# QData/LaMP

Measured on AMD Instinct MI355X. Metric: forward samples/sec, reuters d512 2+2L 4h, higher is better.
Workload: dtype f32

## Files before the change

lamp_amd/csrc/attention_small.hip:

```cpp
#include "lamp_kernels.h"

namespace lamp {

#ifndef LAMP_LDS_PAD16
#define LAMP_LDS_PAD16 8
#endif
constexpr int ATTN16_PAD = LAMP_LDS_PAD16;

namespace {
__device__ __forceinline__ void swap16(float& a, float& b) {
    asm volatile("s_nop 3\n\tv_permlane16_swap_b32 %0, %1\n\ts_nop 3" : "+v"(a), "+v"(b));
}
__device__ __forceinline__ void swap32(float& a, float& b) {
    asm volatile("s_nop 3\n\tv_permlane32_swap_b32 %0, %1\n\ts_nop 3" : "+v"(a), "+v"(b));
}
__device__ __forceinline__ float group_max(float v) {
    float a = v, b = v;
    swap16(a, b);
    a = fmaxf(a, b);
    b = a;
    swap32(a, b);
    return fmaxf(a, b);
}
__device__ __forceinline__ float group_sum(float v) {
    float a = v, b = v;
    swap16(a, b);
    a = a + b;
    b = a;
    swap32(a, b);
    return a + b;
}
}

template <int DP, int QB, int KSPLIT, int PM, int MK>
__global__ __launch_bounds__(QB* KSPLIT * 64, 3) void attn16_kernel(AttnParams p) {
    constexpr int DKC = DP / 16;
    constexpr int DV8 = DP / 16;
    constexpr int QS = DP + ATTN16_PAD;
    extern __shared__ __attribute__((aligned(16))) float smem[];

    const int tid = threadIdx.x;
    const int lane = tid & 63, wave = tid >> 6;
    const int l15 = lane & 15, g = lane >> 4;
    const int rot = (KSPLIT > 1 && p.kv_len) ? int(blockIdx.x % KSPLIT) : 0;
    const int qb = wave / KSPLIT, ks = __builtin_amdgcn_readfirstlane((wave % KSPLIT + KSPLIT - rot) % KSPLIT);
    const int slot = qb * KSPLIT + ks;
#ifdef LAMP_TUNING
    const unsigned long long t_entry = p.trace ? wall_clock64() : 0ull;
    unsigned long long t_loop = 0, t_merge = 0;
#endif
    const int nqg = (p.lq + 16 * QB - 1) / (16 * QB);
    const int item = xcd_remap(blockIdx.x, gridDim.x);
    const int qgrp = item % nqg;
    const int bh = item / nqg;
    const int h = bh % p.H, b = bh / p.H;
    const int q0 = (qgrp * QB + qb) * 16;
    const int qi = q0 + l15;
    const bool wave_active = q0 < p.lq;
    const int qc = qi < p.lq ? qi : p.lq - 1;

    const int q_r = int(p.lay.q_r), k_r = int(p.lay.k_r), v_r = int(p.lay.v_r);
    const int lk_b = __builtin_amdgcn_readfirstlane(p.kv_len ? p.kv_len[b] : p.lk);
    const int row0 = __builtin_amdgcn_readfirstlane(p.kv_len ? p.kv_off[b] : 0);
    const int64_t k_row0 = p.kv_len ? int64_t(row0) * k_r : int64_t(b) * p.lay.k_b;
    const int64_t v_row0 = p.kv_len ? int64_t(row0) * v_r : int64_t(b) * p.lay.v_b;
    const __amdgpu_buffer_rsrc_t rsQ = make_rsrc(p.Q + int64_t(b) * p.lay.q_b + int64_t(h) * p.lay.q_h,
                                                 (uint64_t(p.lq - 1) * q_r + p.dk) * 4u);
    const __amdgpu_buffer_rsrc_t rsK = make_rsrc(p.K + k_row0 + int64_t(h) * p.lay.k_h,
                                                 lk_b > 0 ? (uint64_t(lk_b - 1) * k_r + p.dk) * 4u : 0);
    const __amdgpu_buffer_rsrc_t rsV = make_rsrc(p.V + v_row0 + int64_t(h) * p.lay.v_h,
                                                 lk_b > 0 ? (uint64_t(lk_b - 1) * v_r + p.dv) * 4u : 0);
    const __amdgpu_buffer_rsrc_t rsM =
        MK == LAMP_MASK_BITS_U32
            ? make_rsrc(static_cast<const unsigned*>(p.mask) + int64_t(b) * p.m_sb,
                        (uint64_t(p.lq - 1) * uint64_t(p.m_sq) + (p.lk + 31) / 32) * 4u)
        : MK == LAMP_MASK_U8
            ? make_rsrc(static_cast<const unsigned char*>(p.mask) + int64_t(b) * p.m_sb,
                        uint64_t(p.lq - 1) * uint64_t(p.m_sq) + p.lk)
        : MK == LAMP_MASK_KEY_TOKENS_I64
            ? make_rsrc(static_cast<const long long*>(p.mask) + int64_t(b) * p.m_sb, uint64_t(p.lk) * 8u)
            : make_rsrc(p.K, 0);

    float* Qs = smem + qb * 16 * QS;
    float* Ks = smem + (QB + wave) * 16 * QS;
    {
        constexpr int C4 = DP / 4;
        constexpr int PER_WAVE = 16 * C4 / KSPLIT;
#pragma unroll
        for (int i = 0; i < (PER_WAVE + 63) / 64; ++i) {
            const int idx = ks * PER_WAVE + i * 64 + lane;
            const int row = idx / C4, c = (idx - row * C4) * 4;
            const int q = q0 + row;
            if (i * 64 + lane < PER_WAVE) {
                const float4 v = bload4(rsQ, (q < p.lq && c < p.dk) ? unsigned(q * q_r + c) * 4u : OOB, 0);
                *reinterpret_cast<float4*>(Qs + row * QS + c) =
                    make_float4(v.x * p.scale_log2e, v.y * p.scale_log2e, v.z * p.scale_log2e, v.w * p.scale_log2e);
            }
        }
    }
    __syncthreads();

    const int nt_b = (lk_b + 15) / 16;
    const int nt = PM == 2 ? (p.lk + 15) / 16 : nt_b;
    const int ks_eff = (KSPLIT > 1 && p.kv_len) ? (nt_b >= 12 ? (KSPLIT < 4 ? KSPLIT : 4) : (nt_b >= 4 ? 2 : 1)) : KSPLIT;
    float4 kg[DKC];
    constexpr int C4K = DP / 4, RPI = 64 / C4K;
    float vf[4][DV8];
    unsigned mbits = 0;

    const unsigned k_voff = (lane % C4K) * 4 < p.dk ? unsigned((lane / C4K) * k_r + (lane % C4K) * 4) * 4u : OOB;
    auto load_k = [&](int kt) {
#pragma unroll
        for (int i = 0; i < DKC; ++i) kg[i] = bload4(rsK, k_voff, unsigned((kt * 16 + i * RPI) * k_r) * 4u);
    };
    auto stage_k = [&]() {
        const int c = (lane % C4K) * 4;
#pragma unroll
        for (int i = 0; i < DKC; ++i) *reinterpret_cast<float4*>(Ks + (i * RPI + lane / C4K) * QS + c) = kg[i];
    };
    constexpr int DVW = DV8 == 8 ? 4 : DV8;
    const unsigned v_voff = DVW * l15 < p.dv ? unsigned(4 * g * v_r + DVW * l15) * 4u : OOB;
    const unsigned v_voff2 = 64 + DVW * l15 < p.dv ? unsigned(4 * g * v_r + DVW * l15) * 4u + 256u : OOB;
    auto load_v = [&](int kt) {
#pragma unroll
        for (int r = 0; r < 4; ++r) {
            const unsigned off = v_voff, so = unsigned((kt * 16 + r) * v_r) * 4u;
            if constexpr (DV8 == 8) {
                const float4 a = bload4(rsV, off, so);
                const float4 c2 = bload4(rsV, v_voff2, so);
                vf[r][0] = a.x; vf[r][1] = a.y; vf[r][2] = a.z; vf[r][3] = a.w;
                vf[r][4] = c2.x; vf[r][5] = c2.y; vf[r][6] = c2.z; vf[r][7] = c2.w;
            } else if constexpr (DV8 == 4) {
                const float4 a = bload4(rsV, off, so);
                vf[r][0] = a.x; vf[r][1] = a.y; vf[r][2] = a.z; vf[r][3] = a.w;
            } else {
                const f32x2 a = bload2(rsV, off + so);
                vf[r][0] = a.x; vf[r][1] = a.y;
            }
        }
    };
    const unsigned m_voff = unsigned(int64_t(qc) * p.m_sq) * 4u;
    auto load_mask = [&](int kt) {
        const int kbase = kt * 16 + 4 * g;
        if constexpr (MK == LAMP_MASK_BITS_U32) {
            mbits = __builtin_amdgcn_raw_buffer_load_b32(rsM, m_voff, unsigned(kt >> 1) * 4u, 0);
        } else if constexpr (MK == LAMP_MASK_U8) {
            const unsigned mo = unsigned(int64_t(qc) * p.m_sq) + unsigned(kbase);
            unsigned m = 0;
#pragma unroll
            for (int r = 0; r < 4; ++r) m |= (bload_u8(rsM, kt < nt ? mo + r : OOB) != 0 ? 1u : 0u) << r;
            mbits = m;
        } else if constexpr (MK == LAMP_MASK_KEY_TOKENS_I64) {
            unsigned m = 0;
#pragma unroll
            for (int r = 0; r < 4; ++r)
                m |= (bload_u64(rsM, unsigned(kbase + r) * 8u) == 0 ? 1u : 0u) << r;
            mbits = m;
        }
    };
    auto scores = [&](int kt, f32x4& s) {
        const int valid = lk_b - kt * 16;
        const unsigned tail = valid >= 16 ? 0u : (0xffffu << (valid > 0 ? valid : 0)) & 0xffffu;
        unsigned word = tail;
        if constexpr (MK == LAMP_MASK_BITS_U32) word |= mbits >> ((kt & 1) * 16);
        const int mine = MK == LAMP_MASK_BITS_U32 || MK == LAMP_MASK_NONE ? int(word >> (4 * g)) : int(mbits | (tail >> (4 * g)));
        f32x4 s0, s1 = {0.f, 0.f, 0.f, 0.f};
#pragma unroll
        for (int r = 0; r < 4; ++r) {
            int t;
            asm("v_bfe_i32 %0, %1, %2, 1" : "=v"(t) : "v"(mine), "n"(r));
            s0[r] = __int_as_float(t & int(0xff800000u));
        }
#ifdef LAMP_SETPRIO
        __builtin_amdgcn_s_setprio(1);
#endif
        const float* qp = Qs + l15 * QS + 4 * g;
        const float* kp = Ks + l15 * QS + 4 * g;
#pragma unroll
        for (int c = 0; c < DKC; c += 2) {
            const float4 qa = *reinterpret_cast<const float4*>(qp + 16 * c);
            const float4 qb2 = *reinterpret_cast<const float4*>(qp + 16 * c + 16);
            const float4 ka = *reinterpret_cast<const float4*>(kp + 16 * c);
            const float4 kb = *reinterpret_cast<const float4*>(kp + 16 * c + 16);
            s0 = __builtin_amdgcn_mfma_f32_16x16x4f32(ka.x, qa.x, s0, 0, 0, 0);
            s1 = __builtin_amdgcn_mfma_f32_16x16x4f32(kb.x, qb2.x, s1, 0, 0, 0);
            s0 = __builtin_amdgcn_mfma_f32_16x16x4f32(ka.y, qa.y, s0, 0, 0, 0);
            s1 = __builtin_amdgcn_mfma_f32_16x16x4f32(kb.y, qb2.y, s1, 0, 0, 0);
            s0 = __builtin_amdgcn_mfma_f32_16x16x4f32(ka.z, qa.z, s0, 0, 0, 0);
            s1 = __builtin_amdgcn_mfma_f32_16x16x4f32(kb.z, qb2.z, s1, 0, 0, 0);
            s0 = __builtin_amdgcn_mfma_f32_16x16x4f32(ka.w, qa.w, s0, 0, 0, 0);
            s1 = __builtin_amdgcn_mfma_f32_16x16x4f32(kb.w, qb2.w, s1, 0, 0, 0);
        }
#ifdef LAMP_SETPRIO
        __builtin_amdgcn_s_setprio(0);
#endif
#pragma unroll
        for (int r = 0; r < 4; ++r) s[r] = s0[r] + s1[r];
    };

    f32x4 o[DV8];
#pragma unroll
    for (int e = 0; e < DV8; ++e) o[e] = f32x4{0.f, 0.f, 0.f, 0.f};
    float m_run = -INFINITY, l_part = 0.f;
    constexpr float RESCALE_THR = 32.0f;

#ifdef LAMP_TUNING
    if (p.trace) t_loop = wall_clock64();
#endif
    if (wave_active && ks < ks_eff && ks < nt) {
        int kt = ks;
        load_k(kt);
        load_mask(kt);
        load_v(kt);
        for (; kt < nt; kt += ks_eff) {
            const int kn = kt + ks_eff;
            f32x4 s;
            stage_k();
            scores(kt, s);
            __builtin_amdgcn_sched_barrier(0);
            load_k(kn);
            load_mask(kn);
            if constexpr (PM == 2) {
                float* Srow = p.P + (int64_t(h) * p.P_batch + p.P_b0 + b) * int64_t(p.lq) * p.lk + int64_t(qi) * p.lk;
#pragma unroll
                for (int r = 0; r < 4; ++r) {
                    const int key = kt * 16 + 4 * g + r;
                    if (qi < p.lq && key < p.lk) Srow[key] = s[r];
                }
            }
            const float tmax = fmaxf(fmaxf(s[0], s[1]), fmaxf(s[2], s[3]));
            if (__any(tmax > m_run + RESCALE_THR)) {
                const float m_new = fmaxf(m_run, group_max(tmax));
                const float alpha = __builtin_amdgcn_exp2f(m_run - ((m_new == -INFINITY) ? 0.f : m_new));
                l_part *= alpha;
                m_run = m_new;
#pragma unroll
                for (int e = 0; e < DV8; ++e)
#pragma unroll
                    for (int r = 0; r < 4; ++r) o[e][r] *= alpha;
            }
            const float m_use = (m_run == -INFINITY) ? 0.f : m_run;
#pragma unroll
            for (int r = 0; r < 4; ++r) s[r] = __builtin_amdgcn_exp2f(s[r] - m_use);
            l_part += (s[0] + s[1]) + (s[2] + s[3]);
#ifdef LAMP_SETPRIO
            __builtin_amdgcn_s_setprio(1);
#endif
#pragma unroll
            for (int r = 0; r < 4; ++r)
#pragma unroll
                for (int e = 0; e < DV8; ++e)
                    o[e] = __builtin_amdgcn_mfma_f32_16x16x4f32(vf[r][e], s[r], o[e], 0, 0, 0);
#ifdef LAMP_SETPRIO
            __builtin_amdgcn_s_setprio(0);
#endif
            __builtin_amdgcn_sched_barrier(0);
            load_v(kn);
        }
    }

#ifdef LAMP_TUNING
    if (p.trace) t_merge = wall_clock64();
#endif
    if constexpr (KSPLIT > 1) {
        constexpr int CW = (DV8 * 4 + 4) * 64;
        __syncthreads();
        float* mine = smem + slot * CW;
#pragma unroll
        for (int e = 0; e < DV8; ++e)
            *reinterpret_cast<float4*>(mine + (e * 64 + lane) * 4) = make_float4(o[e][0], o[e][1], o[e][2], o[e][3]);
        *reinterpret_cast<float4*>(mine + (DV8 * 64 + lane) * 4) = make_float4(m_run, l_part, 0.f, 0.f);
        __syncthreads();
        if (ks == 0 && wave_active) {
            float m_all = m_run;
#pragma unroll
            for (int s2 = 1; s2 < KSPLIT; ++s2)
                if (s2 < ks_eff) m_all = fmaxf(m_all, smem[(slot + s2) * CW + (DV8 * 64 + lane) * 4]);
            const float m_use = (m_all == -INFINITY) ? 0.f : m_all;
            const float w0 = exp2f(m_run - m_use);
            l_part *= w0;
#pragma unroll
            for (int e = 0; e < DV8; ++e)
#pragma unroll
                for (int r = 0; r < 4; ++r) o[e][r] *= w0;
#pragma unroll
            for (int s2 = 1; s2 < KSPLIT; ++s2) {
                if (s2 >= ks_eff) break;
                const float* other = smem + (slot + s2) * CW;
                const float4 ml = *reinterpret_cast<const float4*>(other + (DV8 * 64 + lane) * 4);
                const float ws = exp2f(ml.x - m_use);
                l_part = fmaf(ml.y, ws, l_part);
#pragma unroll
                for (int e = 0; e < DV8; ++e) {
                    const float4 v = *reinterpret_cast<const float4*>(other + (e * 64 + lane) * 4);
                    o[e][0] = fmaf(v.x, ws, o[e][0]);
                    o[e][1] = fmaf(v.y, ws, o[e][1]);
                    o[e][2] = fmaf(v.z, ws, o[e][2]);
                    o[e][3] = fmaf(v.w, ws, o[e][3]);
                }
            }
            m_run = m_all;
        }
    }
    if (!(wave_active && ks == 0)) return;
    const float l_run = group_sum(l_part);
    if constexpr (PM == 2) {
        if (g == 0 && qi < p.lq)
            p.lse[(int64_t(h) * p.B + b) * int64_t(p.lq) + qi] = ((m_run == -INFINITY) ? 0.f : m_run) + log2f(l_run);
    }
    const float inv_l = 1.0f / l_run;

    if (qi < p.lq) {
        float* Orow = p.O + int64_t(b) * p.lay.o_b + int64_t(h) * p.lay.o_h + int64_t(qi) * p.lay.o_r;
        const bool vec = ((p.lay.o_b | p.lay.o_h | p.lay.o_r) & 3) == 0 && (reinterpret_cast<uintptr_t>(p.O) & 15u) == 0;
#pragma unroll
        for (int r = 0; r < 4; ++r) {
#pragma unroll
            for (int e0 = 0; e0 < DV8; e0 += DVW) {
                const int col = DVW * (4 * g + r) + 64 * (e0 / DVW);
                if (col >= p.dv) continue;
                if (DVW == 4 && vec) {
                    *reinterpret_cast<float4*>(Orow + col) =
                        make_float4(o[e0][r] * inv_l, o[e0 + (DVW > 1 ? 1 : 0)][r] * inv_l,
                                    o[e0 + (DVW > 2 ? 2 : 0)][r] * inv_l, o[e0 + (DVW > 3 ? 3 : 0)][r] * inv_l);
                } else {
#pragma unroll
                    for (int e = 0; e < DVW; ++e) Orow[col + e] = o[e0 + e][r] * inv_l;
                }
            }
        }
    }
#ifdef LAMP_TUNING
    if (p.trace && tid == 0) {
        unsigned long long* t = p.trace + size_t(blockIdx.x) * 8;
        t[0] = t_entry; t[1] = t_loop; t[2] = t_merge; t[3] = wall_clock64();
        t[4] = __builtin_amdgcn_s_getreg((31 << 11) | 4);
        t[5] = __builtin_amdgcn_s_getreg((31 << 11) | 20);
        t[6] = unsigned(item);
        t[7] = unsigned(ks) | (unsigned(qb) << 8);
    }
#endif
}

template <int DP, int QB, int KSPLIT, int PM, int MK>
static int launch_small_mk(const AttnParams& p, hipStream_t s) {
    constexpr int NW = QB * KSPLIT;
    constexpr size_t lds_q = size_t(QB + NW) * 16 * (DP + ATTN16_PAD) * sizeof(float);
    constexpr size_t lds_c = KSPLIT > 1 ? size_t(NW) * (DP / 16 * 4 + 4) * 64 * sizeof(float) : 0;
    constexpr size_t lds = lds_q > lds_c ? lds_q : lds_c;
    auto kern = attn16_kernel<DP, QB, KSPLIT, PM, MK>;
    if constexpr (lds > 65536) {
        static AttrOnce once;
        if (int e = once.set(reinterpret_cast<const void*>(kern), lds)) return e;
    }
    const int64_t nwg = int64_t((p.lq + 16 * QB - 1) / (16 * QB)) * p.H * p.B;
    if (nwg > 0x7fffffffLL) return LAMP_E_DIMS;
    hipLaunchKernelGGL(kern, dim3(unsigned(nwg)), dim3(NW * 64), lds, s, p);
    return int(hipGetLastError());
}

template <int DP, int QB, int KSPLIT, int PM>
static int launch_small_ks(const AttnParams& p, hipStream_t s) {
    switch (p.mask_kind) {
        case LAMP_MASK_U8: return launch_small_mk<DP, QB, KSPLIT, PM, LAMP_MASK_U8>(p, s);
        case LAMP_MASK_KEY_TOKENS_I64: return launch_small_mk<DP, QB, KSPLIT, PM, LAMP_MASK_KEY_TOKENS_I64>(p, s);
        case LAMP_MASK_BITS_U32: return launch_small_mk<DP, QB, KSPLIT, PM, LAMP_MASK_BITS_U32>(p, s);
        default: return launch_small_mk<DP, QB, KSPLIT, PM, LAMP_MASK_NONE>(p, s);
    }
}

template <int DP, int QB, int KSPLIT>
static int launch_small_pm(const AttnParams& p, hipStream_t s) {
    return p.lse ? launch_small_ks<DP, QB, KSPLIT, 2>(p, s) : launch_small_ks<DP, QB, KSPLIT, 0>(p, s);
}

template <int DP>
static int launch_small_dp(const AttnParams& p, int qb, int ksplit, hipStream_t s) {
    switch (qb * 8 + ksplit) {
        case 1 * 8 + 1: return launch_small_pm<DP, 4, 1>(p, s);
        case 2 * 8 + 1: return launch_small_pm<DP, 4, 1>(p, s);
        case 3 * 8 + 1: return launch_small_pm<DP, 4, 1>(p, s);
        case 4 * 8 + 1: return launch_small_pm<DP, 4, 1>(p, s);
        case 1 * 8 + 2: return launch_small_pm<DP, 2, 2>(p, s);
        case 2 * 8 + 2: return launch_small_pm<DP, 2, 2>(p, s);
        case 3 * 8 + 2: return launch_small_pm<DP, 3, 2>(p, s);
        case 4 * 8 + 2: return launch_small_pm<DP, 4, 2>(p, s);
        case 1 * 8 + 4: return launch_small_pm<DP, 1, 4>(p, s);
        case 2 * 8 + 4: return launch_small_pm<DP, 2, 4>(p, s);
        case 3 * 8 + 4: return launch_small_pm<DP, 3, 4>(p, s);
        default: return launch_small_pm<DP, 2, 4>(p, s);
    }
}

bool attn_small_applies(const AttnParams& p, bool any_lq) {
    const bool few_keys = p.lk <= 64 && !p.kv_len;
    return (p.lq <= 256 || few_keys || any_lq) && p.V && p.O && (!p.P || p.lse) && p.dk <= 128 && p.dv <= 128;
}

#ifdef LAMP_TUNING
static unsigned long long* g_attn_trace = nullptr;
extern "C" __attribute__((visibility("default"))) void lamp_debug_set_attn_trace(unsigned long long* buf) { g_attn_trace = buf; }
#endif

int launch_attn_small(const AttnParams& p_in, int force, hipStream_t s) {
    AttnParams p = p_in;
    p.trace = nullptr;
#ifdef LAMP_TUNING
    p.trace = g_attn_trace;
#endif
    const int nt = (p.lk + 15) / 16;
    const int nqb = (p.lq + 15) / 16;
    int ksplit = force & 7;
    if (ksplit != 1 && ksplit != 2 && ksplit != 4) {
        ksplit = nt >= 12 ? 4 : (nt >= 4 ? 2 : 1);
        if (p.self_ragged && !p.kv_len) ksplit = 1;
    }
    int qb = (force >> 4) & 7;
    if (qb < 1 || qb > 4) qb = 4 / ksplit;
    (void)nqb;
    const int dmax = p.dk > p.dv ? p.dk : p.dv;
    if (dmax <= 32) return launch_small_dp<32>(p, qb, ksplit, s);
    if (dmax <= 64) return launch_small_dp<64>(p, qb, ksplit, s);
    return launch_small_dp<128>(p, qb, ksplit, s);
}

}
```

lamp_amd/csrc/gemm.hip:

```cpp
#include <type_traits>

#include "lamp_kernels.h"

namespace lamp {

struct FastDiv {
    unsigned mul, shift;
};
static inline FastDiv make_fastdiv(unsigned d) {
    if (d <= 1) return FastDiv{0u, 0u};
    unsigned l = 0;
    while ((1ull << l) < d) ++l;
    return FastDiv{unsigned(((1ull << (31 + l)) + d - 1) / d), l - 1};
}
__device__ __forceinline__ int fdiv(int n, FastDiv f) { return f.mul ? int(__umulhi(unsigned(n), f.mul) >> f.shift) : n; }
__device__ __forceinline__ int div_1_to_8(int n, int d) {
    if ((d & (d - 1)) == 0) return n >> (31 - __builtin_clz(unsigned(d)));
    const unsigned mul = d == 5 ? 0xCCCCCCCDu : (d == 7 ? 0x92492493u : 0xAAAAAAABu);
    return int(__umulhi(unsigned(n), mul) >> (d == 3 ? 1 : 2));
}

constexpr int gemm_min_waves(int bm, int bn, int bk, int mf) { return (mf == 16 && bm == 64 && bn == 64 && bk == 16) ? 5 : 1; }

template <int BM, int BN, int BK, int WAVES_M, int WAVES_N, int MF = 32>
struct GemmTile {
    static constexpr int NT = WAVES_M * WAVES_N * 64;
    static constexpr int WTM = BM / WAVES_M;
    static constexpr int WTN = BN / WAVES_N;
    static constexpr int MI = WTM / MF;
    static constexpr int NI = WTN / MF;
#ifndef LAMP_LDS_PAD16
#define LAMP_LDS_PAD16 8
#endif
    static constexpr int LDS_STRIDE = BK + (MF == 16 ? LAMP_LDS_PAD16 : 4);
    static constexpr int A_LD = BM * BK / 4 / NT;
    static constexpr int B_LD = BN * BK / 4 / NT;
    static constexpr size_t LDS_BYTES = size_t(2) * (BM + BN) * LDS_STRIDE * sizeof(float);
    static constexpr int MIN_WAVES = gemm_min_waves(BM, BN, BK, MF);
    static_assert(MF == 32 || MF == 16, "MFMA block edge");
    static_assert(WTM % MF == 0 && WTN % MF == 0, "wave tile must be a multiple of the MFMA block");
    static_assert(BK % (MF == 32 ? 8 : 16) == 0, "BK must cover whole fragment reads");
    static_assert((BM * BK / 4) % NT == 0 && (BN * BK / 4) % NT == 0, "staging must divide evenly");
    static_assert(BK % 8 == 0, "BK must be a multiple of 8");
};


__device__ __forceinline__ const float* uniform_ptr(const float* q) {
    const uint64_t b = reinterpret_cast<uint64_t>(q);
    const unsigned lo = __builtin_amdgcn_readfirstlane(unsigned(b)), hi = __builtin_amdgcn_readfirstlane(unsigned(b >> 32));
    return reinterpret_cast<const float*>((uint64_t(hi) << 32) | lo);
}
template <int BM, int BN, int BK, int WAVES_M, int WAVES_N, bool KTAIL, int MF, bool RPRE, bool VEC, bool RGATHER>
__device__ __forceinline__ void gemm_body(const GemmParams& p, int tiles_n_seg, int tiles_n, int tiles_m, int panel_split,
                                          FastDiv fd_group, FastDiv fd_seg) {
    using T = GemmTile<BM, BN, BK, WAVES_M, WAVES_N, MF>;
    constexpr int KQ = 64 / MF;
    constexpr int KCH = 4 * KQ;
    constexpr int NACC = MF == 32 ? 16 : 4;
    using acc_t = typename std::conditional<MF == 32, f32x16, f32x4>::type;
    constexpr int S = T::LDS_STRIDE;
    constexpr int C4 = BK / 4;
    extern __shared__ __attribute__((aligned(16))) float smem[];
    float* As = smem;
    float* Bs = smem + 2 * BM * S;

    const int tid = threadIdx.x;
    const int lane = tid & 63;
    const int wave = tid >> 6;
    const int wm = wave / WAVES_N, wn = wave % WAVES_N;
    const int l31 = lane & (MF - 1), hi = lane / MF;

#ifdef LAMP_TUNING
    const unsigned long long t_entry = p.trace ? wall_clock64() : 0ull;
#endif
    constexpr int GROUP_M = 8;
    int64_t M = p.M;
    if (p.m_dev) {
        M = *p.m_dev;
        if (M > p.M) M = p.M;
        tiles_m = int((M + BM - 1) / BM);
        const int nwg = tiles_m * tiles_n, pan_xcd = (tiles_m + 7) >> 3;
        panel_split = tiles_m >= 16 && (pan_xcd * tiles_n + 31) / 32 <= ((nwg + 7) / 8 + 31) / 32;
    }
    int item = 0, pan0 = 0, pan1 = tiles_m;
    int tn_all = 0, tm = 0;
    if (panel_split) {
        const int q = tiles_m >> 3, r = tiles_m & 7, xcd = blockIdx.x & 7;
        pan0 = xcd * q + (xcd < r ? xcd : r);
        pan1 = pan0 + q + (xcd < r ? 1 : 0);
        item = blockIdx.x >> 3;
        if (item >= (pan1 - pan0) * tiles_n) return;
    } else {
        const int nwg = p.m_dev ? tiles_m * tiles_n : int(gridDim.x);
        if (int(blockIdx.x) >= nwg) return;
        item = xcd_remap(blockIdx.x, nwg);
        pan0 = 0;
        pan1 = tiles_m;
    }
    if (p.walk_gn > 0) {
        const int rows = pan1 - pan0;
        const int group_sz = rows * p.walk_gn;
        const int grp = item / group_sz;
        const int in_grp = item - grp * group_sz;
        const int first_n = grp * p.walk_gn;
        const int gn = tiles_n - first_n < p.walk_gn ? tiles_n - first_n : p.walk_gn;
        const int tml = in_grp / gn;
        tm = pan0 + tml;
        tn_all = first_n + (in_grp - tml * gn);
    } else {
        const int group_sz = GROUP_M * tiles_n;
        const int grp = fdiv(item, fd_group);
        const int in_grp = item - grp * group_sz;
        const int first_m = pan0 + grp * GROUP_M;
        const int gm = pan1 - first_m < GROUP_M ? pan1 - first_m : GROUP_M;
        tn_all = div_1_to_8(in_grp, gm);
        tm = first_m + (in_grp - tn_all * gm);
    }
    const int seg = fdiv(tn_all, fd_seg);
    const int tn = tn_all - seg * tiles_n_seg;
    const int64_t m0 = int64_t(tm) * BM;
    const int n0 = tn * BN;
    const int rows_m = int(M - m0 < BM ? M - m0 : BM);
    const int rows_n = p.N - n0 < BN ? p.N - n0 : BN;

    const int lda = int(p.lda), ldw = int(p.ldw);
    const float* Abase = p.A;
    if (p.A_dense) {
        if (p.m_dev[0] == p.m_dev[1]) Abase = p.A_dense;
    }
    const __amdgpu_buffer_rsrc_t rsA =
        make_rsrc(uniform_ptr(Abase + m0 * p.lda), __builtin_amdgcn_readfirstlane(unsigned((uint64_t(rows_m - 1) * lda + p.K) * 4u)));
    const __amdgpu_buffer_rsrc_t rsW =
        make_rsrc(uniform_ptr(p.W[seg] + int64_t(n0) * p.ldw), __builtin_amdgcn_readfirstlane(unsigned((uint64_t(rows_n - 1) * ldw + p.K) * 4u)));

    acc_t acc[T::MI][T::NI];
#pragma unroll
    for (int i = 0; i < T::MI; ++i)
#pragma unroll
        for (int j = 0; j < T::NI; ++j)
#pragma unroll
            for (int r = 0; r < NACC; ++r) acc[i][j][r] = 0.f;

    float4 ra0[T::A_LD], rb0[T::B_LD], ra1[T::A_LD], rb1[T::B_LD];
    unsigned voa[T::A_LD], vob[T::B_LD];
#pragma unroll
    for (int i = 0; i < T::A_LD; ++i) {
        const int idx = tid + i * T::NT;
        const int row = idx / C4, c4 = idx - row * C4;
        voa[i] = unsigned(row * lda + c4 * 4) * 4u;
    }
#pragma unroll
    for (int i = 0; i < T::B_LD; ++i) {
        const int idx = tid + i * T::NT;
        const int row = idx / C4, c4 = idx - row * C4;
        vob[i] = unsigned(row * ldw + c4 * 4) * 4u;
    }

    auto gload = [&](int k0, float4 (&ra)[T::A_LD], float4 (&rb)[T::B_LD]) {
        if constexpr (KTAIL) {
#pragma unroll
            for (int i = 0; i < T::A_LD; ++i) {
                const int k = k0 + ((tid + i * T::NT) % C4) * 4;
                ra[i] = bload4(rsA, k < p.K ? voa[i] + unsigned(k0) * 4u : OOB, 0);
            }
#pragma unroll
            for (int i = 0; i < T::B_LD; ++i) {
                const int k = k0 + ((tid + i * T::NT) % C4) * 4;
                rb[i] = bload4(rsW, k < p.K ? vob[i] + unsigned(k0) * 4u : OOB, 0);
            }
        } else {
            const unsigned so = unsigned(k0) * 4u;
#pragma unroll
            for (int i = 0; i < T::A_LD; ++i) ra[i] = bload4(rsA, voa[i], so);
#pragma unroll
            for (int i = 0; i < T::B_LD; ++i) rb[i] = bload4(rsW, vob[i], so);
        }
    };
    auto lstore = [&](int buf, const float4 (&ra)[T::A_LD], const float4 (&rb)[T::B_LD]) {
        float* a = As + buf * BM * S;
        float* b = Bs + buf * BN * S;
#pragma unroll
        for (int i = 0; i < T::A_LD; ++i) {
            const int idx = tid + i * T::NT;
            const int row = idx / C4, c4 = idx - row * C4;
            *reinterpret_cast<float4*>(a + row * S + c4 * 4) = ra[i];
        }
#pragma unroll
        for (int i = 0; i < T::B_LD; ++i) {
            const int idx = tid + i * T::NT;
            const int row = idx / C4, c4 = idx - row * C4;
            *reinterpret_cast<float4*>(b + row * S + c4 * 4) = rb[i];
        }
    };
    auto mfma_chunk = [&](const float4 (&fa)[T::MI], const float4 (&fb)[T::NI]) {
#ifdef LAMP_SETPRIO
        __builtin_amdgcn_s_setprio(1);
#endif
#pragma unroll
        for (int i = 0; i < T::MI; ++i)
#pragma unroll
            for (int j = 0; j < T::NI; ++j) {
                if constexpr (MF == 32) {
                    acc[i][j] = __builtin_amdgcn_mfma_f32_32x32x2f32(fb[j].x, fa[i].x, acc[i][j], 0, 0, 0);
                    acc[i][j] = __builtin_amdgcn_mfma_f32_32x32x2f32(fb[j].y, fa[i].y, acc[i][j], 0, 0, 0);
                    acc[i][j] = __builtin_amdgcn_mfma_f32_32x32x2f32(fb[j].z, fa[i].z, acc[i][j], 0, 0, 0);
                    acc[i][j] = __builtin_amdgcn_mfma_f32_32x32x2f32(fb[j].w, fa[i].w, acc[i][j], 0, 0, 0);
                } else {
                    acc[i][j] = __builtin_amdgcn_mfma_f32_16x16x4f32(fb[j].x, fa[i].x, acc[i][j], 0, 0, 0);
                    acc[i][j] = __builtin_amdgcn_mfma_f32_16x16x4f32(fb[j].y, fa[i].y, acc[i][j], 0, 0, 0);
                    acc[i][j] = __builtin_amdgcn_mfma_f32_16x16x4f32(fb[j].z, fa[i].z, acc[i][j], 0, 0, 0);
                    acc[i][j] = __builtin_amdgcn_mfma_f32_16x16x4f32(fb[j].w, fa[i].w, acc[i][j], 0, 0, 0);
                }
            }
#ifdef LAMP_SETPRIO
        __builtin_amdgcn_s_setprio(0);
#endif
    };
    auto compute = [&](int buf) {
        const float* a = As + buf * BM * S + (wm * T::WTM + l31) * S + hi * 4;
        const float* b = Bs + buf * BN * S + (wn * T::WTN + l31) * S + hi * 4;
#pragma unroll
        for (int c = 0; c < BK / KCH; ++c) {
            float4 fa[T::MI], fb[T::NI];
#pragma unroll
            for (int i = 0; i < T::MI; ++i) fa[i] = *reinterpret_cast<const float4*>(a + i * MF * S + c * KCH);
#pragma unroll
            for (int j = 0; j < T::NI; ++j) fb[j] = *reinterpret_cast<const float4*>(b + j * MF * S + c * KCH);
            mfma_chunk(fa, fb);
        }
    };

    const int nk = (p.K + BK - 1) / BK;
    gload(0, ra0, rb0);

    const int ldc = int(p.ldc), ldr = int(p.ldr);
    const bool has_r = RGATHER || p.R != nullptr;
    const bool read_r = !RGATHER && p.R != nullptr;
    const __amdgpu_buffer_rsrc_t rsR =
        make_rsrc(read_r ? p.R + m0 * p.ldr + n0 : p.A, read_r ? (uint64_t(rows_m - 1) * ldr + rows_n) * 4u : 0);
    const float* bias = p.bias[seg];
    const __amdgpu_buffer_rsrc_t rsBias = make_rsrc(bias ? bias + n0 : p.A, bias ? uint64_t(rows_n) * 4u : 0);
    constexpr int NQ = NACC / 4;
    constexpr bool vec = VEC;
    const int lrow0 = wm * T::WTM + l31;
    const int lcol0 = wn * T::WTN + 4 * hi;
    auto load4 = [&](__amdgpu_buffer_rsrc_t rs, unsigned off, int lcol) -> float4 {
        if constexpr (vec) return bload4(rs, lcol < rows_n ? off * 4u : OOB, 0);
        float4 v;
        v.x = bload1(rs, lcol + 0 < rows_n ? (off + 0) * 4u : OOB);
        v.y = bload1(rs, lcol + 1 < rows_n ? (off + 1) * 4u : OOB);
        v.z = bload1(rs, lcol + 2 < rows_n ? (off + 2) * 4u : OOB);
        v.w = bload1(rs, lcol + 3 < rows_n ? (off + 3) * 4u : OOB);
        return v;
    };
    const float* ge[RGATHER ? T::MI : 1];
    const float* gp[RGATHER ? T::MI : 1];
    if constexpr (RGATHER) {
#pragma unroll
        for (int i = 0; i < T::MI; ++i) {
            const int lrow = lrow0 + i * MF;
            const bool in = lrow < rows_m;
            const int tk = in ? p.rg_tok[m0 + lrow] : 0, ps = (in && p.rg_pos_table) ? p.rg_pos[m0 + lrow] : 0;
            ge[i] = p.rg_emb + int64_t(tk) * p.N + n0;
            gp[i] = p.rg_pos_table ? p.rg_pos_table + int64_t(ps) * p.N + n0 : nullptr;
        }
    }
    auto gathered = [&](int i, int lcol) -> float4 {
        if constexpr (RGATHER) {
            if (lcol >= rows_n) return make_float4(0.f, 0.f, 0.f, 0.f);
            float4 v = *reinterpret_cast<const float4*>(ge[i] + lcol);
            if (gp[i]) {
                const float4 w = *reinterpret_cast<const float4*>(gp[i] + lcol);
                v.x += w.x; v.y += w.y; v.z += w.z; v.w += w.w;
            }
            return v;
        }
        return make_float4(0.f, 0.f, 0.f, 0.f);
    };
    constexpr int NPRE = RPRE ? T::MI * T::NI * NQ : 1;
    float4 pre_r[NPRE], pre_b[RPRE ? T::NI * NQ : 1];
    if constexpr (RPRE) {
#pragma unroll
        for (int j = 0; j < T::NI; ++j)
#pragma unroll
            for (int q = 0; q < NQ; ++q) {
                const int lcol = lcol0 + j * MF + 8 * q;
                pre_b[j * NQ + q] = load4(rsBias, unsigned(lcol), lcol);
#pragma unroll
                for (int i = 0; i < T::MI; ++i)
                    pre_r[(j * T::MI + i) * NQ + q] = RGATHER ? gathered(i, lcol) : load4(rsR, unsigned((lrow0 + i * MF) * ldr + lcol), lcol);
            }
    }

    lstore(0, ra0, rb0);
    if (nk > 1) gload(BK, ra0, rb0);
    if (nk > 2) gload(2 * BK, ra1, rb1);
    __syncthreads();
#ifdef LAMP_TUNING
    const unsigned long long t_loop = p.trace ? wall_clock64() : 0ull;
    const unsigned long long c_loop = p.trace ? __builtin_readcyclecounter() : 0ull;
#endif

    for (int kt = 0; kt < nk; kt += 2) {
        compute(0);
        if (kt + 1 < nk) lstore(1, ra0, rb0);
        if (kt + 3 < nk) gload((kt + 3) * BK, ra0, rb0);
        __syncthreads();
        if (kt + 1 >= nk) break;
        compute(1);
        if (kt + 2 < nk) lstore(0, ra1, rb1);
        if (kt + 4 < nk) gload((kt + 4) * BK, ra1, rb1);
        __syncthreads();
    }
#ifdef LAMP_TUNING
    const unsigned long long t_epi = p.trace ? wall_clock64() : 0ull;
    const unsigned long long c_epi = p.trace ? __builtin_readcyclecounter() : 0ull;
#endif

    const __amdgpu_buffer_rsrc_t rsC =
        make_rsrc(p.C[seg] + m0 * p.ldc + n0, (uint64_t(rows_m - 1) * ldc + rows_n) * 4u);
    auto relu1 = [](float x) {
        float y;
        asm("v_max_f32 %0, 0, %1" : "=v"(y) : "v"(x));
        return y;
    };
    auto emit = [&](auto with_r, auto with_relu) {
        constexpr bool WITH_R = decltype(with_r)::value, WITH_RELU = decltype(with_relu)::value;
    #pragma unroll
        for (int i = 0; i < T::MI; ++i) {
            const int lrow = lrow0 + i * MF;
    #pragma unroll
            for (int j = 0; j < T::NI; ++j)
    #pragma unroll
                for (int q = 0; q < NQ; ++q) {
                    const int lcol = lcol0 + j * MF + 8 * q;
                    float4 bv, res = make_float4(0.f, 0.f, 0.f, 0.f);
                    if constexpr (RPRE) {
                        bv = pre_b[j * NQ + q];
                        res = pre_r[(j * T::MI + i) * NQ + q];
                    } else {
                        bv = load4(rsBias, unsigned(lcol), lcol);
                        if constexpr (WITH_R) res = RGATHER ? gathered(i, lcol) : load4(rsR, unsigned(lrow * ldr + lcol), lcol);
                    }
                    float4 v = make_float4(acc[i][j][4 * q + 0] + bv.x, acc[i][j][4 * q + 1] + bv.y,
                                           acc[i][j][4 * q + 2] + bv.z, acc[i][j][4 * q + 3] + bv.w);
                    if constexpr (WITH_RELU) v = make_float4(relu1(v.x), relu1(v.y), relu1(v.z), relu1(v.w));
                    if constexpr (WITH_R) v = make_float4(v.x + res.x, v.y + res.y, v.z + res.z, v.w + res.w);
                    const unsigned off = unsigned(lrow * ldc + lcol);
                    if constexpr (vec) {
                        bstore4(rsC, lcol < rows_n ? off * 4u : OOB, v);
                    } else {
                        bstore1(rsC, lcol + 0 < rows_n ? (off + 0) * 4u : OOB, v.x);
                        bstore1(rsC, lcol + 1 < rows_n ? (off + 1) * 4u : OOB, v.y);
                        bstore1(rsC, lcol + 2 < rows_n ? (off + 2) * 4u : OOB, v.z);
                        bstore1(rsC, lcol + 3 < rows_n ? (off + 3) * 4u : OOB, v.w);
                    }
                }
        }
    };
    if (has_r) {
        if (p.relu) emit(std::true_type{}, std::true_type{});
        else emit(std::true_type{}, std::false_type{});
    } else {
        if (p.relu) emit(std::false_type{}, std::true_type{});
        else emit(std::false_type{}, std::false_type{});
    }
#ifdef LAMP_TUNING
    if (p.trace && tid == 0) {
        unsigned long long* t = p.trace + size_t(blockIdx.x) * 8;
        t[0] = t_entry; t[1] = t_loop; t[2] = t_epi; t[3] = wall_clock64();
        t[4] = __builtin_amdgcn_s_getreg((31 << 11) | 4);
        t[5] = __builtin_amdgcn_s_getreg((31 << 11) | 20);
        t[6] = unsigned(item);
        t[7] = c_epi - c_loop;
    }
#endif
}

template <int BM, int BN, int BK, int WAVES_M, int WAVES_N, bool KTAIL, int MF, bool RPRE, bool VEC, bool RGATHER = false>
__global__ __launch_bounds__(WAVES_M* WAVES_N * 64, (gemm_min_waves(BM, BN, BK, MF))) void gemm_nt_kernel(GemmParams p, int tiles_n_seg,
                                                                          int tiles_n, int tiles_m,
                                                                          int panel_split, FastDiv fd_group,
                                                                          FastDiv fd_seg) {
    gemm_body<BM, BN, BK, WAVES_M, WAVES_N, KTAIL, MF, RPRE, VEC, RGATHER>(p, tiles_n_seg, tiles_n, tiles_m, panel_split, fd_group, fd_seg);
}

#ifdef LAMP_TUNING
static int g_force_walk = -1;
extern "C" __attribute__((visibility("default"))) void lamp_debug_force_gemm_walk(int gn) { g_force_walk = gn; }
static long long g_trace_slab_words = 0;
static size_t g_extra_lds = 0;
extern "C" __attribute__((visibility("default"))) void lamp_debug_set_gemm_extra_lds(int bytes) { g_extra_lds = size_t(bytes); }
#endif

template <int BM, int BN, int BK, int WAVES_M, int WAVES_N, bool KTAIL, int MF, bool VEC, bool RGATHER = false>
static int launch_cfg2(const GemmParams& p, hipStream_t s) {
    using T = GemmTile<BM, BN, BK, WAVES_M, WAVES_N, MF>;
    constexpr bool RPRE = T::MI * T::NI * (MF == 32 ? 16 : 4) <= 16;
    auto kern = gemm_nt_kernel<BM, BN, BK, WAVES_M, WAVES_N, KTAIL, MF, RPRE, VEC, RGATHER>;
    size_t LDS = T::LDS_BYTES;
    static AttrOnce once;
#ifdef LAMP_TUNING
    LDS += g_extra_lds;
    if (int e = once.set(reinterpret_cast<const void*>(kern), 160 * 1024)) return e;
#else
    if (int e = once.set(reinterpret_cast<const void*>(kern), LDS)) return e;
#endif
    const int64_t ldmax = p.lda > p.ldw ? (p.lda > p.ldc ? p.lda : p.ldc) : (p.ldw > p.ldc ? p.ldw : p.ldc);
    if (ldmax * (BM > BN ? BM : BN) * 4 >= 0x7fffffffLL || (p.R && p.ldr * BM * 4 >= 0x7fffffffLL))
        return LAMP_E_UNSUPPORTED;
    const int64_t tiles_m = (p.M + BM - 1) / BM;
    const int tiles_n_seg = (p.N + BN - 1) / BN;
    const int tiles_n = tiles_n_seg * p.nseg;
    int64_t nwg = tiles_m * tiles_n;
    const int64_t pan_xcd = (tiles_m + 7) / 8;
    int panel_split = tiles_m >= 16 && (pan_xcd * tiles_n + 31) / 32 <= ((nwg + 7) / 8 + 31) / 32;
    if (panel_split) nwg = 8 * pan_xcd * tiles_n;
    if (p.m_dev) {
        const int64_t split_grid = 8 * pan_xcd * tiles_n;
        if (split_grid > nwg) nwg = split_grid;
        panel_split = 0;
    }
    if (nwg > 0x7fffffffLL) return LAMP_E_DIMS;
    GemmParams q = p;
    q.walk_gn = (int64_t(p.nseg) * p.N * p.K * 4 >= (8ll << 20) && tiles_n > 8) ? 8 : 0;
#ifdef LAMP_TUNING
    if (p.trace && nwg * 8 > g_trace_slab_words) return LAMP_E_WORKSPACE;
    if (g_force_walk >= 0) q.walk_gn = g_force_walk < tiles_n ? g_force_walk : tiles_n;
#endif
    hipLaunchKernelGGL(kern, dim3((unsigned)nwg), dim3(T::NT), LDS, s, q, tiles_n_seg, tiles_n, int(tiles_m),
                       panel_split, make_fastdiv(unsigned(8 * tiles_n)), make_fastdiv(unsigned(tiles_n_seg)));
    return int(hipGetLastError());
}

template <int BM, int BN, int BK, int WAVES_M, int WAVES_N, int MF = 32>
static int launch_cfg(const GemmParams& p, hipStream_t s) {
    if (p.rg_tok) {
        if (!p.vec_epilogue || (p.K % BK)) return LAMP_E_UNSUPPORTED;
        return launch_cfg2<BM, BN, BK, WAVES_M, WAVES_N, false, MF, true, true>(p, s);
    }
    if (p.vec_epilogue) {
        if (p.K % BK) return launch_cfg2<BM, BN, BK, WAVES_M, WAVES_N, true, MF, true>(p, s);
        return launch_cfg2<BM, BN, BK, WAVES_M, WAVES_N, false, MF, true>(p, s);
    }
    if (p.K % BK) return launch_cfg2<BM, BN, BK, WAVES_M, WAVES_N, true, MF, false>(p, s);
    return launch_cfg2<BM, BN, BK, WAVES_M, WAVES_N, false, MF, false>(p, s);
}

#ifdef LAMP_TUNING
static int g_force_tile = 0;
static unsigned long long* g_gemm_trace = nullptr;
static long long g_trace_slab = 0;
static int g_trace_slabs = 0, g_trace_count = 0;
extern "C" __attribute__((visibility("default"))) void lamp_debug_force_gemm_tile(int cfg) { g_force_tile = cfg; }
extern "C" __attribute__((visibility("default"))) void lamp_debug_set_gemm_trace(unsigned long long* buf, long long slab_words, int n_slabs) {
    g_gemm_trace = buf;
    g_trace_slab = slab_words;
    g_trace_slab_words = slab_words;
    g_trace_slabs = n_slabs;
    g_trace_count = 0;
}
#endif

bool gemm_gathered_residual_ok(int N, int K, int64_t ldc, const float* bias, const float* C, const float* emb, const float* pos_table) {
    return N > 0 && !(N & 3) && K > 0 && (K % 32) == 0 && !(ldc & 3) && aligned16(C) && (!bias || aligned16(bias)) && emb && aligned16(emb) &&
           (!pos_table || aligned16(pos_table));
}

int launch_gemm(const GemmParams& p_in, hipStream_t s) {
    GemmParams p = p_in;
    if (p.M <= 0 || p.N <= 0 || p.K <= 0 || p.nseg < 1 || p.nseg > GEMM_MAX_SEG) return LAMP_E_DIMS;
    if ((p.K & 3) || (p.lda & 3) || (p.ldw & 3)) return LAMP_E_ALIGN;
    if (!p.A || (p.A_dense && !p.m_dev)) return LAMP_E_NULL;
    if (p.rg_tok && (p.R || !p.rg_emb || p.nseg != 1 || (p.rg_pos_table && !p.rg_pos))) return LAMP_E_UNSUPPORTED;
    if (p.rg_tok && (!aligned16(p.rg_emb) || (p.rg_pos_table && !aligned16(p.rg_pos_table)))) return LAMP_E_ALIGN;
    if (!aligned16(p.A) || (p.A_dense && !aligned16(p.A_dense))) return LAMP_E_ALIGN;
    for (int i = 0; i < p.nseg; ++i) {
        if (!p.W[i] || !p.C[i]) return LAMP_E_NULL;
        if (!aligned16(p.W[i])) return LAMP_E_ALIGN;
    }
    const double flops = 2.0 * double(p.M) * p.N * p.nseg * p.K;
    const double bytes = 4.0 * (double(p.M) * p.K + double(p.N) * p.nseg * p.K +
                                double(p.M) * p.N * p.nseg * ((p.R || p.rg_tok) ? 2 : 1));
    ProfScope prof(LAMP_K_GEMM, flops, bytes, s);
    p.trace = nullptr;
    bool vec = !(p.N & 3) && !(p.ldc & 3) && (!p.R || (!(p.ldr & 3) && aligned16(p.R)));
    for (int i = 0; i < p.nseg; ++i) vec = vec && aligned16(p.C[i]) && (!p.bias[i] || aligned16(p.bias[i]));
    p.vec_epilogue = vec ? 1 : 0;
#ifdef LAMP_TUNING
    if (g_gemm_trace && g_trace_slabs > 0) {
        const long long wg_max = ((p.M + 31) / 32) * ((p.N + 63) / 64) * p.nseg;
        if (wg_max * 8 <= g_trace_slab) p.trace = g_gemm_trace + (g_trace_count % g_trace_slabs) * g_trace_slab;
        ++g_trace_count;
    }
    switch (g_force_tile) {
        case 1: return launch_cfg<128, 128, 32, 2, 2>(p, s);
        case 2: return launch_cfg<64, 64, 32, 2, 2>(p, s);
        case 3: return launch_cfg<128, 64, 32, 2, 2>(p, s);
        case 4: return launch_cfg<64, 128, 32, 2, 2>(p, s);
        case 5: return launch_cfg<128, 128, 16, 2, 2>(p, s);
        case 6: return launch_cfg<64, 64, 16, 2, 2>(p, s);
        case 7: return launch_cfg<128, 64, 16, 2, 2>(p, s);
        case 8: return launch_cfg<256, 128, 16, 4, 2>(p, s);
        case 9: return launch_cfg<32, 64, 32, 1, 4, 16>(p, s);
        case 10: return launch_cfg<64, 32, 32, 4, 1, 16>(p, s);
        case 11: return launch_cfg<64, 64, 16, 2, 2, 16>(p, s);
        case 12: return launch_cfg<64, 64, 32, 2, 2, 16>(p, s);
        case 13: return launch_cfg<32, 128, 32, 1, 4, 16>(p, s);
        case 14: return launch_cfg<128, 128, 32, 2, 2, 16>(p, s);
        case 15: return launch_cfg<128, 128, 16, 2, 2, 16>(p, s);
        case 16: return launch_cfg<128, 64, 32, 2, 2, 16>(p, s);
        case 17: return launch_cfg<64, 128, 32, 2, 2, 16>(p, s);
        case 18: return launch_cfg<128, 64, 16, 2, 2, 16>(p, s);
        default: break;
    }
#endif
    auto tiles = [&](int bm, int bn) { return ((p.M + bm - 1) / bm) * ((p.N + bn - 1) / bn) * p.nseg; };
    const int64_t t64 = tiles(64, 64);
    if (tiles(128, 64) >= 2048 && p.K >= 512) return launch_cfg<128, 64, 16, 2, 2, 16>(p, s);
    if (t64 >= 2048) return launch_cfg<64, 64, 32, 2, 2, 16>(p, s);
    if (t64 >= 1200) return launch_cfg<64, 64, 16, 2, 2, 16>(p, s);
    return launch_cfg<32, 64, 32, 1, 4, 16>(p, s);
}

}
```

Baseline: 46420.

## Overlap prologue loads in attention and GEMM kernels to hide latency

In the small attention kernel, the Q tile global loads, the first K/V tile loads and the mask request are now all issued before the scaled Q is written to LDS and the block synchronises. The mask fold is split from its load so the first tile's mask latency overlaps too. In the GEMM, the first two K-slices are prefetched into separate register buffers before the bias/residual/gather prologue, and the embedding and position gathers are issued as separate batches, so more memory requests are in flight at once. The cost is higher register pressure in both kernels, which may reduce occupancy.

```diff
diff --git a/lamp_amd/csrc/attention_small.hip b/lamp_amd/csrc/attention_small.hip
--- a/lamp_amd/csrc/attention_small.hip
+++ b/lamp_amd/csrc/attention_small.hip
@@ -83,22 +83,6 @@
 
     float* Qs = smem + qb * 16 * QS;
     float* Ks = smem + (QB + wave) * 16 * QS;
-    {
-        constexpr int C4 = DP / 4;
-        constexpr int PER_WAVE = 16 * C4 / KSPLIT;
-#pragma unroll
-        for (int i = 0; i < (PER_WAVE + 63) / 64; ++i) {
-            const int idx = ks * PER_WAVE + i * 64 + lane;
-            const int row = idx / C4, c = (idx - row * C4) * 4;
-            const int q = q0 + row;
-            if (i * 64 + lane < PER_WAVE) {
-                const float4 v = bload4(rsQ, (q < p.lq && c < p.dk) ? unsigned(q * q_r + c) * 4u : OOB, 0);
-                *reinterpret_cast<float4*>(Qs + row * QS + c) =
-                    make_float4(v.x * p.scale_log2e, v.y * p.scale_log2e, v.z * p.scale_log2e, v.w * p.scale_log2e);
-            }
-        }
-    }
-    __syncthreads();
 
     const int nt_b = (lk_b + 15) / 16;
     const int nt = PM == 2 ? (p.lk + 15) / 16 : nt_b;
@@ -140,23 +124,33 @@
         }
     };
     const unsigned m_voff = unsigned(int64_t(qc) * p.m_sq) * 4u;
-    auto load_mask = [&](int kt) {
+    constexpr bool MASK_RAW = MK == LAMP_MASK_U8 || MK == LAMP_MASK_KEY_TOKENS_I64;
+    typename std::conditional<MK == LAMP_MASK_KEY_TOKENS_I64, unsigned long long, unsigned>::type mraw[MASK_RAW ? 4 : 1];
+    auto request_mask = [&](int kt) {
         const int kbase = kt * 16 + 4 * g;
         if constexpr (MK == LAMP_MASK_BITS_U32) {
             mbits = __builtin_amdgcn_raw_buffer_load_b32(rsM, m_voff, unsigned(kt >> 1) * 4u, 0);
         } else if constexpr (MK == LAMP_MASK_U8) {
             const unsigned mo = unsigned(int64_t(qc) * p.m_sq) + unsigned(kbase);
+#pragma unroll
+            for (int r = 0; r < 4; ++r) mraw[r] = bload_u8(rsM, kt < nt ? mo + r : OOB);
+        } else if constexpr (MK == LAMP_MASK_KEY_TOKENS_I64) {
+#pragma unroll
+            for (int r = 0; r < 4; ++r)
+                mraw[r] = bload_u64(rsM, unsigned(kbase + r) * 8u);
+        }
+    };
+    auto fold_mask = [&]() {
+        if constexpr (MASK_RAW) {
             unsigned m = 0;
 #pragma unroll
-            for (int r = 0; r < 4; ++r) m |= (bload_u8(rsM, kt < nt ? mo + r : OOB) != 0 ? 1u : 0u) << r;
+            for (int r = 0; r < 4; ++r) m |= ((MK == LAMP_MASK_U8 ? mraw[r] != 0 : mraw[r] == 0) ? 1u : 0u) << r;
             mbits = m;
-        } else if constexpr (MK == LAMP_MASK_KEY_TOKENS_I64) {
-            unsigned m = 0;
-#pragma unroll
-            for (int r = 0; r < 4; ++r)
-                m |= (bload_u64(rsM, unsigned(kbase + r) * 8u) == 0 ? 1u : 0u) << r;
-            mbits = m;
-        }
+        }
+    };
+    auto load_mask = [&](int kt) {
+        request_mask(kt);
+        fold_mask();
     };
     auto scores = [&](int kt, f32x4& s) {
         const int valid = lk_b - kt * 16;
@@ -204,14 +198,42 @@
     float m_run = -INFINITY, l_part = 0.f;
     constexpr float RESCALE_THR = 32.0f;
 
+    const bool has_tile = wave_active && ks < ks_eff && ks < nt;
+    {
+        constexpr int C4 = DP / 4;
+        constexpr int PER_WAVE = 16 * C4 / KSPLIT;
+        constexpr int NQL = (PER_WAVE + 63) / 64;
+        float4 qv[NQL];
+#pragma unroll
+        for (int i = 0; i < NQL; ++i) {
+            const int idx = ks * PER_WAVE + i * 64 + lane;
+            const int row = idx / C4, c = (idx - row * C4) * 4;
+            const int q = q0 + row;
+            if (i * 64 + lane < PER_WAVE) qv[i] = bload4(rsQ, (q < p.lq && c < p.dk) ? unsigned(q * q_r + c) * 4u : OOB, 0);
+        }
+        __builtin_amdgcn_sched_barrier(0);
+        if (has_tile) {
+            load_k(ks);
+            request_mask(ks);
+            load_v(ks);
+        }
+        __builtin_amdgcn_sched_barrier(0);
+#pragma unroll
+        for (int i = 0; i < NQL; ++i) {
+            const int idx = ks * PER_WAVE + i * 64 + lane;
+            const int row = idx / C4, c = (idx - row * C4) * 4;
+            if (i * 64 + lane < PER_WAVE)
+                *reinterpret_cast<float4*>(Qs + row * QS + c) =
+                    make_float4(qv[i].x * p.scale_log2e, qv[i].y * p.scale_log2e, qv[i].z * p.scale_log2e, qv[i].w * p.scale_log2e);
+        }
+    }
+    __syncthreads();
 #ifdef LAMP_TUNING
     if (p.trace) t_loop = wall_clock64();
 #endif
-    if (wave_active && ks < ks_eff && ks < nt) {
+    if (has_tile) {
         int kt = ks;
-        load_k(kt);
-        load_mask(kt);
-        load_v(kt);
+        fold_mask();
         for (; kt < nt; kt += ks_eff) {
             const int kn = kt + ks_eff;
             f32x4 s;
diff --git a/lamp_amd/csrc/gemm.hip b/lamp_amd/csrc/gemm.hip
--- a/lamp_amd/csrc/gemm.hip
+++ b/lamp_amd/csrc/gemm.hip
@@ -123,6 +123,18 @@
     const int rows_m = int(M - m0 < BM ? M - m0 : BM);
     const int rows_n = p.N - n0 < BN ? p.N - n0 : BN;
 
+    const int lrow0 = wm * T::WTM + l31;
+    int rg_tk[RGATHER ? T::MI : 1], rg_ps[RGATHER ? T::MI : 1];
+    if constexpr (RGATHER) {
+#pragma unroll
+        for (int i = 0; i < T::MI; ++i) {
+            const int lrow = lrow0 + i * MF;
+            const bool in = lrow < rows_m;
+            rg_tk[i] = in ? p.rg_tok[m0 + lrow] : 0;
+            rg_ps[i] = (in && p.rg_pos_table) ? p.rg_pos[m0 + lrow] : 0;
+        }
+    }
+
     const int lda = int(p.lda), ldw = int(p.ldw);
     const float* Abase = p.A;
     if (p.A_dense) {
@@ -232,6 +244,8 @@
 
     const int nk = (p.K + BK - 1) / BK;
     gload(0, ra0, rb0);
+    if (nk > 1) gload(BK, ra1, rb1);
+    __builtin_amdgcn_sched_barrier(0);
 
     const int ldc = int(p.ldc), ldr = int(p.ldr);
     const bool has_r = RGATHER || p.R != nullptr;
@@ -242,7 +256,6 @@
     const __amdgpu_buffer_rsrc_t rsBias = make_rsrc(bias ? bias + n0 : p.A, bias ? uint64_t(rows_n) * 4u : 0);
     constexpr int NQ = NACC / 4;
     constexpr bool vec = VEC;
-    const int lrow0 = wm * T::WTM + l31;
     const int lcol0 = wn * T::WTN + 4 * hi;
     auto load4 = [&](__amdgpu_buffer_rsrc_t rs, unsigned off, int lcol) -> float4 {
         if constexpr (vec) return bload4(rs, lcol < rows_n ? off * 4u : OOB, 0);
@@ -258,11 +271,8 @@
     if constexpr (RGATHER) {
 #pragma unroll
         for (int i = 0; i < T::MI; ++i) {
-            const int lrow = lrow0 + i * MF;
-            const bool in = lrow < rows_m;
-            const int tk = in ? p.rg_tok[m0 + lrow] : 0, ps = (in && p.rg_pos_table) ? p.rg_pos[m0 + lrow] : 0;
-            ge[i] = p.rg_emb + int64_t(tk) * p.N + n0;
-            gp[i] = p.rg_pos_table ? p.rg_pos_table + int64_t(ps) * p.N + n0 : nullptr;
+            ge[i] = p.rg_emb + int64_t(rg_tk[i]) * p.N + n0;
+            gp[i] = p.rg_pos_table ? p.rg_pos_table + int64_t(rg_ps[i]) * p.N + n0 : nullptr;
         }
     }
     auto gathered = [&](int i, int lcol) -> float4 {
@@ -278,7 +288,7 @@
         return make_float4(0.f, 0.f, 0.f, 0.f);
     };
     constexpr int NPRE = RPRE ? T::MI * T::NI * NQ : 1;
-    float4 pre_r[NPRE], pre_b[RPRE ? T::NI * NQ : 1];
+    float4 pre_r[NPRE], pre_b[RPRE ? T::NI * NQ : 1], pre_p[RPRE && RGATHER ? NPRE : 1];
     if constexpr (RPRE) {
 #pragma unroll
         for (int j = 0; j < T::NI; ++j)
@@ -287,14 +297,41 @@
                 const int lcol = lcol0 + j * MF + 8 * q;
                 pre_b[j * NQ + q] = load4(rsBias, unsigned(lcol), lcol);
 #pragma unroll
-                for (int i = 0; i < T::MI; ++i)
-                    pre_r[(j * T::MI + i) * NQ + q] = RGATHER ? gathered(i, lcol) : load4(rsR, unsigned((lrow0 + i * MF) * ldr + lcol), lcol);
-            }
-    }
-
+                for (int i = 0; i < T::MI; ++i) {
+                    const int e = (j * T::MI + i) * NQ + q;
+                    if constexpr (RGATHER) {
+                        pre_r[e] = lcol < rows_n ? *reinterpret_cast<const float4*>(ge[i] + lcol) : make_float4(0.f, 0.f, 0.f, 0.f);
+                    } else {
+                        pre_r[e] = load4(rsR, unsigned((lrow0 + i * MF) * ldr + lcol), lcol);
+                    }
+                }
+            }
+        if constexpr (RGATHER) {
+            if (p.rg_pos_table) {
+#pragma unroll
+                for (int j = 0; j < T::NI; ++j)
+#pragma unroll
+                    for (int q = 0; q < NQ; ++q)
+#pragma unroll
+                        for (int i = 0; i < T::MI; ++i) {
+                            const int lcol = lcol0 + j * MF + 8 * q;
+                            pre_p[(j * T::MI + i) * NQ + q] =
+                                lcol < rows_n ? *reinterpret_cast<const float4*>(gp[i] + lcol) : make_float4(0.f, 0.f, 0.f, 0.f);
+                        }
+            }
+        }
+    }
+
+    if constexpr (RPRE && RGATHER) {
+        if (p.rg_pos_table) {
+#pragma unroll
+            for (int e = 0; e < NPRE; ++e) {
+                pre_r[e].x += pre_p[e].x; pre_r[e].y += pre_p[e].y; pre_r[e].z += pre_p[e].z; pre_r[e].w += pre_p[e].w;
+            }
+        }
+    }
     lstore(0, ra0, rb0);
-    if (nk > 1) gload(BK, ra0, rb0);
-    if (nk > 2) gload(2 * BK, ra1, rb1);
+    if (nk > 2) gload(2 * BK, ra0, rb0);
     __syncthreads();
 #ifdef LAMP_TUNING
     const unsigned long long t_loop = p.trace ? wall_clock64() : 0ull;
@@ -303,13 +340,13 @@
 
     for (int kt = 0; kt < nk; kt += 2) {
         compute(0);
-        if (kt + 1 < nk) lstore(1, ra0, rb0);
-        if (kt + 3 < nk) gload((kt + 3) * BK, ra0, rb0);
+        if (kt + 1 < nk) lstore(1, ra1, rb1);
+        if (kt + 3 < nk) gload((kt + 3) * BK, ra1, rb1);
         __syncthreads();
         if (kt + 1 >= nk) break;
         compute(1);
-        if (kt + 2 < nk) lstore(0, ra1, rb1);
-        if (kt + 4 < nk) gload((kt + 4) * BK, ra1, rb1);
+        if (kt + 2 < nk) lstore(0, ra0, rb0);
+        if (kt + 4 < nk) gload((kt + 4) * BK, ra0, rb0);
         __syncthreads();
     }
 #ifdef LAMP_TUNING
```

After: 46330 (median of 2 runs). About the same (-0.2%).
